# TheCacophonyProject/classifier-pipeline

Hardware: AMD Instinct MI355X
Metric: CPTV frames/s end-to-end (track+classify) at 160x120 (higher is better)
Workload: dtype u16/i32 track stage (f32 normalise, f64 gates); f32 crop/tile; f32 CNN (stride-1 3x3 convs of stages 2-4 (+ the stride-2 one): two fp16 planes per operand rounded to nearest (11 + 11 significand bits), power-of-two range scaling, 3 fp16 MFMAs per K step, device-side rerun in the exact split if an ac

## Files before the change

classifier-pipeline_amd/csrc/cpx_assoc.hip:

```cpp
#include <hip/hip_runtime.h>
#include <cstdlib>

#include "cpx_assoc_core.h"
#include "cpx_final_core.h"
#include "cpx_kernels.h"

namespace cpx {

__global__ __launch_bounds__(64) void cpx_assoc_kernel(AssocArgs a) {
  const int b = blockIdx.x * blockDim.x + threadIdx.x;
  if (b >= a.B) return;
  const int pbase = a.proc_off[b];
  const int nproc = a.proc_off[b + 1] - pbase;
  const int first = a.clip_first[b];
  AssocClip c;
  c.p = &a.params;
  c.cap = a.cap;
  c.max_active = a.params.max_active_tracks;
  c.max_tracks = a.params.max_tracks;
  c.pool = a.pool + (size_t)first * c.max_active;
  c.active = a.active + (size_t)b * c.max_active;
  c.n_active = 0;
  c.tracks = a.tracks + (size_t)b * c.max_tracks;
  c.n_tracks = 0;
  c.next_id = 1;
  c.regs = a.regs + (size_t)b * a.cap;
  c.scores = a.scores + (size_t)b * a.cap * c.max_active;
  c.used = a.used + (size_t)b * a.cap;
  c.status = 0;
  if (!a.fresh) {
    const AssocResume r = a.resume[b];
    c.n_active = r.n_active;
    c.n_tracks = r.n_tracks;
    c.next_id = r.next_id;
    c.status = r.status;
  }
  for (int t = a.t_begin; t < nproc; ++t) {
    const int fidx = a.proc_idx[pbase + t];
    const cpx_frame_info& fi = a.info[fidx];
    int nreg = 0;
    if (a.proc_ffc[pbase + t]) {
      c.n_active = 0;
    } else {
      if (fi.status != 0) c.status = fi.status;
      const int ncomp = fi.status == 0 ? fi.n_components : 0;
      nreg = build_regions(c, a.comps + (size_t)fidx * a.cap, ncomp, t, t > 0);
      if (a.regions_out)
        for (int i = 0; i < nreg; ++i) a.regions_out[(size_t)fidx * a.cap + i] = c.regs[i];
      assoc_frame(c, nreg, t);
    }
    if (a.region_counts) a.region_counts[fidx] = nreg;
  }
  a.n_tracks[b] = c.status != 0 ? 0 : c.n_tracks;
  a.status[b] = c.status;
  AssocResume r;
  r.n_active = c.n_active;
  r.n_tracks = c.n_tracks;
  r.next_id = c.next_id;
  r.status = c.status;
  a.resume[b] = r;
}

__global__ __launch_bounds__(64) void cpx_finalize_kernel(FinalArgs a) {
  const int b = blockIdx.x * blockDim.x + threadIdx.x;
  if (b >= a.B) return;
  const int pbase = a.proc_off[b];
  const int first = a.clip_first[b];
  const int ma = a.params.max_active_tracks, mt = a.params.max_tracks_per_clip;
  FinalScratch sc;
  sc.d = a.scratch_d + (size_t)b * 2 * a.max_frames;
  sc.f = a.scratch_f + (size_t)b * a.max_frames;
  finalize_clip(a.params, a.pool + (size_t)first * ma, a.tracks + (size_t)b * mt, a.n_tracks[b], a.proc_ffc + pbase,
                a.square_width, a.summaries + (size_t)b * mt, a.counts + 4 * b, sc);
}

__global__ __launch_bounds__(1024) void cpx_counts_prefix_kernel(const int* __restrict__ counts, int B, int* __restrict__ prefix) {
  __shared__ int s_wave[16][4];
  __shared__ int s_carry[4];
  const int tid = threadIdx.x, lane = tid & 63, wave = tid >> 6;
  if (tid < 4) s_carry[tid] = 0;
  __syncthreads();
  for (int base = 0; base < B; base += 1024) {
    const int b = base + tid;
    int v[4], inc[4];
#pragma unroll
    for (int k = 0; k < 4; ++k) {
      v[k] = b < B ? counts[4 * b + k] : 0;
      inc[k] = v[k];
#pragma unroll
      for (int d = 1; d < 64; d <<= 1) {
        const int o = __shfl_up(inc[k], d, 64);
        if (lane >= d) inc[k] += o;
      }
      if (lane == 63) s_wave[wave][k] = inc[k];
    }
    __syncthreads();
#pragma unroll
    for (int k = 0; k < 4; ++k) {
      int before = s_carry[k];
      for (int w = 0; w < wave; ++w) before += s_wave[w][k];
      if (b < B) prefix[4 * b + k] = before + inc[k] - v[k];
    }
    __syncthreads();
    if (tid < 4) {
      int tot = s_carry[tid];
      for (int w = 0; w < 16; ++w) tot += s_wave[w][tid];
      s_carry[tid] = tot;
    }
    __syncthreads();
  }
  if (tid < 4) prefix[4 * B + tid] = s_carry[tid];
}

__global__ __launch_bounds__(64) void cpx_plan_kernel(FinalArgs a) {
  const int b = blockIdx.x * blockDim.x + threadIdx.x;
  if (b >= a.B) return;
  const int pbase = a.proc_off[b];
  const int first = a.clip_first[b];
  const int ma = a.params.max_active_tracks, mt = a.params.max_tracks_per_clip;
  plan_clip(a.params, a.pool + (size_t)first * ma, a.summaries + (size_t)b * mt, a.n_tracks[b], a.proc_ffc + pbase,
            a.proc_idx + pbase, a.square_width, b, a.prefix + 4 * b, a.refs, a.track_offsets, a.reqs, a.sample_track,
            a.track_clip, reinterpret_cast<unsigned char*>(a.scratch_d + (size_t)b * 2 * a.max_frames), b == a.B - 1);
}

static inline int lanes_per_wave(int B) {
  int l = B / 2048;
  return l < 1 ? 1 : (l > 64 ? 64 : l);
}

void launch_finalize(const FinalArgs& a, hipStream_t s) {
  const int l = lanes_per_wave(a.B);
  hipLaunchKernelGGL(cpx_finalize_kernel, dim3((a.B + l - 1) / l), dim3(l), 0, s, a);
}
void launch_counts_prefix(const int* counts, int B, int* prefix, hipStream_t s) {
  hipLaunchKernelGGL(cpx_counts_prefix_kernel, dim3(1), dim3(1024), 0, s, counts, B, prefix);
}
void launch_plan(const FinalArgs& a, hipStream_t s) {
  const int l = lanes_per_wave(a.B);
  hipLaunchKernelGGL(cpx_plan_kernel, dim3((a.B + l - 1) / l), dim3(l), 0, s, a);
}

size_t assoc_active_bytes() { return sizeof(ActiveTrack); }
size_t assoc_score_bytes() { return sizeof(ScoreRec); }

void launch_assoc(const AssocArgs& a, hipStream_t s) {
  const int l = lanes_per_wave(a.B);
  hipLaunchKernelGGL(cpx_assoc_kernel, dim3((a.B + l - 1) / l), dim3(l), 0, s, a);
}

}
```

Baseline: 3.081 million.

## Stage association state and per-frame components in LDS with cooperative group loads

The association kernel now assigns a group of lanes to each clip instead of one lane per clip. The group cooperatively loads windows of up to 16 frames' metadata and their components into LDS. Active tracks and region buffers are also kept in LDS when they fit a per-group budget. Lane 0 of each group then runs the serial build_regions/assoc_frame on the LDS copies. The aim is to replace scattered serial global loads with coalesced group loads and faster LDS access. In exchange, most lanes now sit idle during the serial phase, fewer clips run per wave, and block-wide barriers are added.

```diff
diff --git a/classifier-pipeline_amd/csrc/cpx_assoc.hip b/classifier-pipeline_amd/csrc/cpx_assoc.hip
--- a/classifier-pipeline_amd/csrc/cpx_assoc.hip
+++ b/classifier-pipeline_amd/csrc/cpx_assoc.hip
@@ -7,58 +7,150 @@
 
 namespace cpx {
 
-__global__ __launch_bounds__(64) void cpx_assoc_kernel(AssocArgs a) {
-  const int b = blockIdx.x * blockDim.x + threadIdx.x;
-  if (b >= a.B) return;
-  const int pbase = a.proc_off[b];
-  const int nproc = a.proc_off[b + 1] - pbase;
-  const int first = a.clip_first[b];
+struct AssocStage {
+  int group;
+  int active, comps, regs;
+  unsigned group_bytes;
+};
+static_assert(sizeof(ActiveTrack) % 8 == 0 && sizeof(RegionRec) % 8 == 0 && sizeof(cpx_component) == 32, "LDS layout");
+#ifndef CPX_ASSOC_LDS_BYTES
+#define CPX_ASSOC_LDS_BYTES 20480
+#endif
+enum { AW_FRAMES = 16 };
+enum { AW_HEAD_BYTES = ((5 * AW_FRAMES + 2) * 4 + 15) & ~15 };
+
+__global__ __launch_bounds__(64) void cpx_assoc_kernel(AssocArgs a, AssocStage st) {
+  extern __shared__ __align__(16) unsigned char smem[];
+  const int lane = threadIdx.x, G = st.group;
+  const int g = lane / G, sub = lane - g * G;
+  const int b = blockIdx.x * (64 / G) + g;
+  const bool live = b < a.B;
+  const int ma = a.params.max_active_tracks;
+  unsigned char* base = smem + (size_t)g * st.group_bytes;
+  int* s_fidx = reinterpret_cast<int*>(base);
+  int* s_ffc = s_fidx + AW_FRAMES;
+  int* s_stat = s_ffc + AW_FRAMES;
+  int* s_nc = s_stat + AW_FRAMES;
+  int* s_off = s_nc + AW_FRAMES;
+  int* s_lw = s_off + AW_FRAMES + 1;
+  unsigned char* q = base + AW_HEAD_BYTES;
+  cpx_component* s_comp = reinterpret_cast<cpx_component*>(q);
+  if (st.comps) q += (size_t)a.cap * sizeof(cpx_component);
+  ActiveTrack* s_act = reinterpret_cast<ActiveTrack*>(q);
+  if (st.active) q += ((size_t)ma * sizeof(ActiveTrack) + 15) & ~(size_t)15;
+  RegionRec* s_regs = reinterpret_cast<RegionRec*>(q);
+  unsigned char* s_used = q + (size_t)a.cap * sizeof(RegionRec);
+
+  int pbase = 0, nproc = 0;
   AssocClip c;
   c.p = &a.params;
   c.cap = a.cap;
-  c.max_active = a.params.max_active_tracks;
+  c.max_active = ma;
   c.max_tracks = a.params.max_tracks;
-  c.pool = a.pool + (size_t)first * c.max_active;
-  c.active = a.active + (size_t)b * c.max_active;
   c.n_active = 0;
-  c.tracks = a.tracks + (size_t)b * c.max_tracks;
   c.n_tracks = 0;
   c.next_id = 1;
-  c.regs = a.regs + (size_t)b * a.cap;
-  c.scores = a.scores + (size_t)b * a.cap * c.max_active;
-  c.used = a.used + (size_t)b * a.cap;
   c.status = 0;
-  if (!a.fresh) {
-    const AssocResume r = a.resume[b];
-    c.n_active = r.n_active;
-    c.n_tracks = r.n_tracks;
-    c.next_id = r.next_id;
-    c.status = r.status;
-  }
-  for (int t = a.t_begin; t < nproc; ++t) {
-    const int fidx = a.proc_idx[pbase + t];
-    const cpx_frame_info& fi = a.info[fidx];
-    int nreg = 0;
-    if (a.proc_ffc[pbase + t]) {
-      c.n_active = 0;
-    } else {
-      if (fi.status != 0) c.status = fi.status;
-      const int ncomp = fi.status == 0 ? fi.n_components : 0;
-      nreg = build_regions(c, a.comps + (size_t)fidx * a.cap, ncomp, t, t > 0);
-      if (a.regions_out)
-        for (int i = 0; i < nreg; ++i) a.regions_out[(size_t)fidx * a.cap + i] = c.regs[i];
-      assoc_frame(c, nreg, t);
-    }
-    if (a.region_counts) a.region_counts[fidx] = nreg;
-  }
-  a.n_tracks[b] = c.status != 0 ? 0 : c.n_tracks;
-  a.status[b] = c.status;
-  AssocResume r;
-  r.n_active = c.n_active;
-  r.n_tracks = c.n_tracks;
-  r.next_id = c.next_id;
-  r.status = c.status;
-  a.resume[b] = r;
+  ActiveTrack* g_act = nullptr;
+  if (live) {
+    pbase = a.proc_off[b];
+    nproc = a.proc_off[b + 1] - pbase;
+    g_act = a.active + (size_t)b * ma;
+    c.pool = a.pool + (size_t)a.clip_first[b] * ma;
+    c.active = st.active ? s_act : g_act;
+    c.tracks = a.tracks + (size_t)b * c.max_tracks;
+    c.regs = st.regs ? s_regs : a.regs + (size_t)b * a.cap;
+    c.scores = a.scores + (size_t)b * a.cap * ma;
+    c.used = st.regs ? s_used : a.used + (size_t)b * a.cap;
+    if (!a.fresh) {
+      const AssocResume r = a.resume[b];
+      c.n_active = r.n_active;
+      c.n_tracks = r.n_tracks;
+      c.next_id = r.next_id;
+      c.status = r.status;
+      if (st.active) {
+        const int words = imin(c.n_active, ma) * (int)(sizeof(ActiveTrack) / 4);
+        const int* src = reinterpret_cast<const int*>(g_act);
+        int* dst = reinterpret_cast<int*>(s_act);
+        for (int i = sub; i < words; i += G) dst[i] = src[i];
+      }
+    }
+  }
+  __syncthreads();
+  int t = a.t_begin;
+  for (;;) {
+    const bool act = live && t < nproc;
+    if (__ballot(act) == 0) break;
+    const int nw = act ? imin((int)AW_FRAMES, nproc - t) : 0;
+    for (int j = sub; j < nw; j += G) {
+      const int fidx = a.proc_idx[pbase + t + j];
+      const int ffc = a.proc_ffc[pbase + t + j];
+      const int status = a.info[fidx].status, ncomp = a.info[fidx].n_components;
+      s_fidx[j] = fidx;
+      s_ffc[j] = ffc;
+      s_stat[j] = status;
+      s_nc[j] = (ffc || status != 0) ? 0 : imin(imax(ncomp, 0), a.cap);
+    }
+    __syncthreads();
+    if (act && sub == 0) {
+      int o = 0, j = 0;
+      for (; j < nw; ++j) {
+        if (j > 0 && o + s_nc[j] > a.cap) break;
+        s_off[j] = o;
+        o += s_nc[j];
+      }
+      s_off[j] = o;
+      *s_lw = j;
+    }
+    __syncthreads();
+    const int lw = act ? *s_lw : 0;
+    if (st.comps && act) {
+      const int total = s_off[lw];
+      for (int e = sub; e < total; e += G) {
+        int j = 0;
+        while (j + 1 < lw && s_off[j + 1] <= e) ++j;
+        s_comp[e] = a.comps[(size_t)s_fidx[j] * a.cap + (e - s_off[j])];
+      }
+    }
+    __syncthreads();
+    if (act && sub == 0) {
+      for (int j = 0; j < lw; ++j) {
+        const int fidx = s_fidx[j], tt = t + j;
+        int nreg = 0;
+        if (s_ffc[j]) {
+          c.n_active = 0;
+        } else {
+          if (s_stat[j] != 0) c.status = s_stat[j];
+          const cpx_component* comps = st.comps ? s_comp + s_off[j] : a.comps + (size_t)fidx * a.cap;
+          nreg = build_regions(c, comps, s_nc[j], tt, tt > 0);
+          if (a.regions_out)
+            for (int i = 0; i < nreg; ++i) a.regions_out[(size_t)fidx * a.cap + i] = c.regs[i];
+          assoc_frame(c, nreg, tt);
+        }
+        if (a.region_counts) a.region_counts[fidx] = nreg;
+      }
+    }
+    __syncthreads();
+    t += lw;
+  }
+  if (live && sub == 0) {
+    a.n_tracks[b] = c.status != 0 ? 0 : c.n_tracks;
+    a.status[b] = c.status;
+    AssocResume r;
+    r.n_active = c.n_active;
+    r.n_tracks = c.n_tracks;
+    r.next_id = c.next_id;
+    r.status = c.status;
+    a.resume[b] = r;
+    *s_lw = c.n_active;
+  }
+  __syncthreads();
+  if (live && st.active) {
+    const int words = imin(*s_lw, ma) * (int)(sizeof(ActiveTrack) / 4);
+    const int* src = reinterpret_cast<const int*>(s_act);
+    int* dst = reinterpret_cast<int*>(g_act);
+    for (int i = sub; i < words; i += G) dst[i] = src[i];
+  }
 }
 
 __global__ __launch_bounds__(64) void cpx_finalize_kernel(FinalArgs a) {
@@ -144,8 +236,22 @@
 size_t assoc_score_bytes() { return sizeof(ScoreRec); }
 
 void launch_assoc(const AssocArgs& a, hipStream_t s) {
-  const int l = lanes_per_wave(a.B);
-  hipLaunchKernelGGL(cpx_assoc_kernel, dim3((a.B + l - 1) / l), dim3(l), 0, s, a);
-}
-
-}
+  AssocStage st{};
+  const int cpw = lanes_per_wave(a.B);
+  int group = 64;
+  while (group * cpw > 64) group >>= 1;
+  st.group = group;
+  const size_t budget = (size_t)CPX_ASSOC_LDS_BYTES / (64 / group);
+  size_t bytes = AW_HEAD_BYTES;
+  const size_t act = ((size_t)a.params.max_active_tracks * sizeof(ActiveTrack) + 15) & ~(size_t)15;
+  const size_t comps = (size_t)a.cap * sizeof(cpx_component);
+  const size_t regs = ((size_t)a.cap * (sizeof(RegionRec) + 1) + 15) & ~(size_t)15;
+  if (bytes + act <= budget) st.active = 1, bytes += act;
+  if (bytes + comps <= budget) st.comps = 1, bytes += comps;
+  if (bytes + regs <= budget) st.regs = 1, bytes += regs;
+  st.group_bytes = (unsigned)bytes;
+  const int per = 64 / group;
+  hipLaunchKernelGGL(cpx_assoc_kernel, dim3((a.B + per - 1) / per), dim3(64), bytes * per, s, a, st);
+}
+
+}
```

Measured after the change: 3.086 million (median of 6 runs). No clear change (+0.2%).
